# showlab/VideoSwap

Measured on NVIDIA H100. Metric: denoise-steps/sec, 16f 512^2 SD1.5 UNet3D (CFG UNet fwd + CFG combine + DDIM step), higher is better.
Workload: dtype f16

## Files before the change

### videoswap_b200/csrc/attention_tc.cu

```cuda
#include "common.cuh"
#include "kernels.h"

namespace vs {
namespace {

constexpr int TQ = 64;
constexpr int ATT_THREADS = 384;
constexpr int PRODUCER_REGS = 24, CONSUMER_REGS = 240;

template <int D>
struct TCfg {
  static constexpr int BKV = 128;
  static constexpr int STAGES = D > 64 ? 3 : 4;
  static constexpr int NCB = (D + 63) / 64;
  static constexpr int DPK = (D + 15) / 16 * 16;
  static constexpr int Q_BLOCK = TQ * 128;
  static constexpr int KV_BLOCK = BKV * 128;
  static constexpr int Q_BYTES = NCB * Q_BLOCK;
  static constexpr int KV_STAGE_BYTES = 2 * NCB * KV_BLOCK;
  static constexpr int OREG = (D > 64) ? 32 + 8 : 32;
  static constexpr int SMEM = 2 * Q_BYTES + STAGES * KV_STAGE_BYTES + 1024 + 8 * (1 + 2 * STAGES);
  static_assert(D == 40 || D == 80, "head dims of the tensor-core path");
  static_assert(SMEM <= 227 * 1024, "shared memory");
};

struct TAttnArgs {
  CUtensorMap tmQ, tmK, tmV;
  __half* o;
  int ldo;
  long long o_bs;
  int nq, nk, kv_div;
  float scale_log2;
};

__device__ __forceinline__ float fast_exp2(float x) {
  float y;
  asm("ex2.approx.ftz.f32 %0, %1;" : "=f"(y) : "f"(x));
  return y;
}
__device__ __forceinline__ uint32_t pack_h2(float a, float b) {
  const __half2 h = __floats2half2_rn(a, b);
  return *reinterpret_cast<const uint32_t*>(&h);
}

template <int D>
__global__ void __launch_bounds__(ATT_THREADS, 1) attn_tc_kernel(const __grid_constant__ TAttnArgs p) {
  using C = TCfg<D>;
  constexpr int BKV = C::BKV, STAGES = C::STAGES;
  extern __shared__ uint8_t smem_raw[];
  const uint32_t base = (smem_u32(smem_raw) + 1023u) & ~1023u;
  const uint32_t q_s = base;
  const uint32_t kv_s = q_s + 2 * C::Q_BYTES;
  const uint32_t bars = kv_s + STAGES * C::KV_STAGE_BYTES;
  const uint32_t q_full = bars;
  auto kv_full = [&](int s) { return bars + 8u * (1 + s); };
  auto kv_empty = [&](int s) { return bars + 8u * (1 + STAGES + s); };

  const int warp = threadIdx.x >> 5, lane = threadIdx.x & 31, wg = threadIdx.x >> 7;
  const int q0 = blockIdx.x * 2 * TQ, head = blockIdx.y, b = blockIdx.z;
  const int nkt = (p.nk + BKV - 1) / BKV;

  if (threadIdx.x == 0) {
    prefetch_tmap(&p.tmQ); prefetch_tmap(&p.tmK); prefetch_tmap(&p.tmV);
    mbar_init(q_full, 1);
    for (int s = 0; s < STAGES; ++s) {
      mbar_init(kv_full(s), 1);
      mbar_init(kv_empty(s), 8);
    }
    fence_barrier_init();
  }
  __syncthreads();
  pdl_trigger();
  pdl_wait();

  if (wg == 0) {
    setmaxnreg_dec<PRODUCER_REGS>();
    if (warp != 0) return;
    const int bk = b / p.kv_div;
    if (elect_one()) {
      mbar_expect_tx(q_full, 2 * C::Q_BYTES);
#pragma unroll
      for (int g = 0; g < 2; ++g)
#pragma unroll
        for (int cb = 0; cb < C::NCB; ++cb)
          tma_load_4d(q_s + g * C::Q_BYTES + cb * C::Q_BLOCK, &p.tmQ, q_full, cb * 64, head, q0 + g * TQ, b);
    }
    __syncwarp();
    for (int j = 0, s = 0, ph = 0; j < nkt; ++j) {
      mbar_wait(kv_empty(s), ph ^ 1);
      if (elect_one()) {
        const uint32_t k_dst = kv_s + s * C::KV_STAGE_BYTES, v_dst = k_dst + C::NCB * C::KV_BLOCK;
        mbar_expect_tx(kv_full(s), C::KV_STAGE_BYTES);
#pragma unroll
        for (int cb = 0; cb < C::NCB; ++cb) {
          tma_load_4d(k_dst + cb * C::KV_BLOCK, &p.tmK, kv_full(s), cb * 64, head, j * BKV, bk);
          tma_load_4d(v_dst + cb * C::KV_BLOCK, &p.tmV, kv_full(s), cb * 64, head, j * BKV, bk);
        }
      }
      __syncwarp();
      if (++s == STAGES) { s = 0; ph ^= 1; }
    }
    return;
  }

  setmaxnreg_inc<CONSUMER_REGS>();
  const int g = wg - 1, wq = warp & 3, q4 = lane & 3;
  const uint32_t qg = q_s + g * C::Q_BYTES;
  const int bar_mine = 1 + g, bar_other = 2 - g;
  if (g == 1) named_bar_arrive(bar_other, 256);

  const float sc = p.scale_log2;
  float o[C::OREG];
#pragma unroll
  for (int i = 0; i < C::OREG; ++i) o[i] = 0.f;
  float m[2] = {-INFINITY, -INFINITY}, l[2] = {0.f, 0.f};
  float s[BKV / 2];
  uint32_t pf[BKV / 16][4];

  auto stage_addr = [&](int j) { return kv_s + (uint32_t)(j % STAGES) * C::KV_STAGE_BYTES; };
  auto issue_qk = [&](int j) {
    const uint32_t k_a = stage_addr(j);
#pragma unroll
    for (int k = 0; k < C::DPK / 16; ++k) {
      const uint32_t qoff = (uint32_t)((k * 16) / 64) * C::Q_BLOCK + (uint32_t)((k * 16) % 64) * 2;
      const uint32_t koff = (uint32_t)((k * 16) / 64) * C::KV_BLOCK + (uint32_t)((k * 16) % 64) * 2;
      wgmma_ss<BKV>(s, gmma_desc_sw128(qg + qoff), gmma_desc_sw128(k_a + koff), k != 0 ? 1u : 0u);
    }
  };
  auto issue_pv = [&](int j) {
    const uint32_t v_a = stage_addr(j) + C::NCB * C::KV_BLOCK;
#pragma unroll
    for (int kk = 0; kk < BKV / 16; ++kk) {
      const uint32_t v_rows = v_a + kk * 16 * 128;
      wgmma_m64n64_rs<1>(o, pf[kk], gmma_desc_sw128_mn(v_rows, C::KV_BLOCK), 1u);
      if (D > 64) wgmma_m64n16_rs<1>(o + 32, pf[kk], gmma_desc_sw128_mn(v_rows + C::KV_BLOCK, C::KV_BLOCK), 1u);
    }
  };
  auto softmax = [&](int j, float* alpha) {
    const int kbase = j * BKV;
    if (kbase + BKV > p.nk) {
#pragma unroll
      for (int i = 0; i < BKV / 2; ++i)
        if (kbase + 8 * (i >> 2) + 2 * q4 + (i & 1) >= p.nk) s[i] = -INFINITY;
    }
#pragma unroll
    for (int h = 0; h < 2; ++h) {
      float mx = m[h];
#pragma unroll
      for (int i = 2 * h; i < BKV / 2; i += 4) mx = fmaxf(mx, fmaxf(s[i], s[i + 1]));
      mx = fmaxf(mx, __shfl_xor_sync(0xffffffffu, mx, 1));
      mx = fmaxf(mx, __shfl_xor_sync(0xffffffffu, mx, 2));
      alpha[h] = fast_exp2((m[h] - mx) * sc);
      m[h] = mx;
      const float ms = mx * sc;
      float rs = 0.f;
#pragma unroll
      for (int i = 2 * h; i < BKV / 2; i += 4) {
        s[i] = fast_exp2(fmaf(s[i], sc, -ms));
        s[i + 1] = fast_exp2(fmaf(s[i + 1], sc, -ms));
        rs += s[i] + s[i + 1];
      }
      l[h] = fmaf(l[h], alpha[h], rs);
    }
  };
  auto pack_p = [&]() {
#pragma unroll
    for (int kk = 0; kk < BKV / 16; ++kk)
#pragma unroll
      for (int r = 0; r < 4; ++r) pf[kk][r] = pack_h2(s[8 * kk + 2 * r], s[8 * kk + 2 * r + 1]);
  };
  auto release = [&](int j) {
    if (lane == 0) mbar_arrive(kv_empty(j % STAGES));
  };

  mbar_wait(q_full, 0);
  mbar_wait(kv_full(0), 0);
  named_bar_sync(bar_mine, 256);
  wgmma_fence();
  issue_qk(0);
  wgmma_commit();
  named_bar_arrive(bar_other, 256);
  wgmma_wait<0>();
  {
    float alpha[2];
    softmax(0, alpha);
    pack_p();
  }
  for (int j = 1; j < nkt; ++j) {
    mbar_wait(kv_full(j % STAGES), (j / STAGES) & 1);
    named_bar_sync(bar_mine, 256);
    wgmma_fence();
    issue_qk(j);
    wgmma_commit();
    issue_pv(j - 1);
    wgmma_commit();
    named_bar_arrive(bar_other, 256);
    wgmma_wait<1>();
    float alpha[2];
    softmax(j, alpha);
    if (p.kv_div > 0) wgmma_wait<0>();
    release(j - 1);
#pragma unroll
    for (int i = 0; i < C::OREG; ++i) o[i] *= alpha[(i >> 1) & 1];
    pack_p();
  }
  named_bar_sync(bar_mine, 256);
  wgmma_fence();
  issue_pv(nkt - 1);
  wgmma_commit();
  if (g == 0) named_bar_arrive(bar_other, 256);
  wgmma_wait<0>();
  release(nkt - 1);

#pragma unroll
  for (int h = 0; h < 2; ++h) {
    l[h] += __shfl_xor_sync(0xffffffffu, l[h], 1);
    l[h] += __shfl_xor_sync(0xffffffffu, l[h], 2);
  }
  const float inv[2] = {1.f / l[0], 1.f / l[1]};
  const int r0 = q0 + g * TQ + 16 * wq + (lane >> 2);
  __half* ob = p.o + b * p.o_bs + head * D;
#pragma unroll
  for (int i = 0; i < C::OREG; i += 2) {
    const int h = (i >> 1) & 1, c = 8 * (i >> 2) + 2 * q4, r = r0 + 8 * h;
    if (c < D && r < p.nq)
      *reinterpret_cast<__half2*>(ob + (long long)r * p.ldo + c) = __floats2half2_rn(o[i] * inv[h], o[i + 1] * inv[h]);
  }
}

template <int D>
int launch(cudaStream_t st, const __half* q, int ldq, const __half* k, int ldk, const __half* v, int ldv, __half* o, int ldo,
           int batch, int nq, int nk, int heads, long long q_bs, long long kv_bs, long long o_bs, int kv_div) {
  using C = TCfg<D>;
  static bool configured = false;
  if (!configured) {
    VS_CHECK_CUDA(cudaFuncSetAttribute(attn_tc_kernel<D>, cudaFuncAttributeMaxDynamicSharedMemorySize, C::SMEM));
    configured = true;
  }
  TAttnArgs a;
  memset(&a, 0, sizeof(a));
  const int bkv = (batch + kv_div - 1) / kv_div;
  {
    const uint64_t dims[4] = {(uint64_t)D, (uint64_t)heads, (uint64_t)nq, (uint64_t)batch};
    const uint64_t str[3] = {(uint64_t)D * 2, (uint64_t)ldq * 2, (uint64_t)(q_bs > 0 ? q_bs : (long long)nq * ldq) * 2};
    const uint32_t box[4] = {64, 1, TQ, 1};
    if (make_tmap_f16(&a.tmQ, q, 4, dims, str, box, 1)) return 3;
  }
  {
    const uint64_t dims[4] = {(uint64_t)D, (uint64_t)heads, (uint64_t)nk, (uint64_t)bkv};
    const uint64_t strk[3] = {(uint64_t)D * 2, (uint64_t)ldk * 2, (uint64_t)(kv_bs > 0 ? kv_bs : (long long)nk * ldk) * 2};
    const uint64_t strv[3] = {(uint64_t)D * 2, (uint64_t)ldv * 2, (uint64_t)(kv_bs > 0 ? kv_bs : (long long)nk * ldv) * 2};
    const uint32_t box[4] = {64, 1, (uint32_t)C::BKV, 1};
    if (make_tmap_f16(&a.tmK, k, 4, dims, strk, box, 1)) return 3;
    if (make_tmap_f16(&a.tmV, v, 4, dims, strv, box, 1)) return 3;
  }
  a.o = o; a.ldo = ldo; a.o_bs = o_bs; a.nq = nq; a.nk = nk; a.kv_div = kv_div;
  a.scale_log2 = 1.4426950408889634f / sqrtf((float)D);
  ProfScope prof(st, PC_ATTN, 4.0 * batch * heads * (double)nq * nk * D, 1, nq, nk, D);
  dim3 grid((nq + 2 * TQ - 1) / (2 * TQ), heads, batch);
  return launch_pdl(attn_tc_kernel<D>, grid, dim3(ATT_THREADS), C::SMEM, st, 1, a);
}

}

int attention_tc(cudaStream_t st, const __half* q, int ldq, const __half* k, int ldk, const __half* v, int ldv, __half* o,
                 int ldo, int batch, int nq, int nk, int heads, int d, long long q_bs, long long kv_bs, long long o_bs,
                 int kv_div) {
  if ((ldq % 8) || (ldk % 8) || (ldv % 8) || (ldo % 2)) return -1;
  if ((q_bs % 8) || (kv_bs % 8)) return -1;
  VS_REQUIRE(kv_div >= 1, "attention_tc: kv_div must be >= 1 (got %d)", kv_div);
  if (d == 40) return launch<40>(st, q, ldq, k, ldk, v, ldv, o, ldo, batch, nq, nk, heads, q_bs, kv_bs, o_bs, kv_div);
  if (d == 80) return launch<80>(st, q, ldq, k, ldk, v, ldv, o, ldo, batch, nq, nk, heads, q_bs, kv_bs, o_bs, kv_div);
  return -1;
}

}
```

### videoswap_b200/csrc/common.cuh

```cuda
#pragma once
#include <cuda.h>
#include <cuda_fp16.h>
#include <cuda_runtime.h>
#include <stdint.h>
#include <stdio.h>

namespace vs {

void set_error(const char* fmt, ...);
const char* last_error();

#define VS_CHECK_CUDA(expr)                                                                         \
  do {                                                                                              \
    cudaError_t _e = (expr);                                                                        \
    if (_e != cudaSuccess) {                                                                        \
      vs::set_error("%s:%d CUDA error %s: %s", __FILE__, __LINE__, #expr, cudaGetErrorString(_e)); \
      return 1;                                                                                     \
    }                                                                                               \
  } while (0)

#define VS_REQUIRE(cond, ...)                \
  do {                                       \
    if (!(cond)) {                           \
      vs::set_error(__VA_ARGS__);            \
      return 2;                              \
    }                                        \
  } while (0)

int make_tmap_f16(CUtensorMap* out, const void* base, int rank, const uint64_t* dims, const uint64_t* strides_bytes,
                  const uint32_t* box, int swizzle );

int num_sms();
int get_option(const char* name);

#ifdef __CUDACC__
template <typename... KArgs, typename... Args>
int launch_pdl(void (*kernel)(KArgs...), dim3 grid, dim3 block, size_t smem, cudaStream_t st, int cluster_x, Args&&... args) {
  cudaLaunchConfig_t cfg = {};
  cfg.gridDim = grid;
  cfg.blockDim = block;
  cfg.dynamicSmemBytes = smem;
  cfg.stream = st;
  cudaLaunchAttribute attr[2];
  int n = 0;
  if (get_option("pdl") != 0) {
    attr[n].id = cudaLaunchAttributeProgrammaticStreamSerialization;
    attr[n].val.programmaticStreamSerializationAllowed = 1;
    ++n;
  }
  if (cluster_x > 1) {
    attr[n].id = cudaLaunchAttributeClusterDimension;
    attr[n].val.clusterDim.x = cluster_x;
    attr[n].val.clusterDim.y = 1;
    attr[n].val.clusterDim.z = 1;
    ++n;
  }
  cfg.attrs = attr;
  cfg.numAttrs = n;
  VS_CHECK_CUDA(cudaLaunchKernelEx(&cfg, kernel, static_cast<KArgs>(args)...));
  return 0;
}
#endif

enum ProfCat { PC_GEMM = 0, PC_CONV = 1, PC_ATTN = 2, PC_TATTN = 3, PC_GROUPNORM = 4, PC_LAYERNORM = 5, PC_OTHER = 6, PC_COUNT = 7 };
struct ProfScope {
  ProfScope(cudaStream_t st, int cat, double work, int nlaunch = 1, long long m = 0, int n = 0, int k = 0);
  ~ProfScope();
  cudaStream_t st_; int idx_;
};
void prof_enable(bool on);
void prof_reset();
int prof_collect(int cat, double* ms, double* work, long long* count);
int prof_dump(const char* path);
long long launch_count();
void count_launch(int n);

#ifdef __CUDACC__
__device__ __forceinline__ uint32_t smem_u32(const void* p) { return (uint32_t)__cvta_generic_to_shared(p); }

__device__ __forceinline__ void mbar_init(uint32_t bar, uint32_t count) {
  asm volatile("mbarrier.init.shared::cta.b64 [%0], %1;" ::"r"(bar), "r"(count) : "memory");
}
__device__ __forceinline__ void fence_barrier_init() {
  asm volatile("fence.mbarrier_init.release.cluster;" ::: "memory");
}
__device__ __forceinline__ void fence_proxy_async() { asm volatile("fence.proxy.async.shared::cta;" ::: "memory"); }
__device__ __forceinline__ void mbar_expect_tx(uint32_t bar, uint32_t bytes) {
  asm volatile("mbarrier.arrive.expect_tx.shared::cta.b64 _, [%0], %1;" ::"r"(bar), "r"(bytes) : "memory");
}
__device__ __forceinline__ void mbar_arrive(uint32_t bar) {
  asm volatile("mbarrier.arrive.shared::cta.b64 _, [%0];" ::"r"(bar) : "memory");
}
__device__ __forceinline__ bool mbar_try_wait(uint32_t bar, uint32_t parity) {
  uint32_t ok;
  asm volatile(
      "{\n\t.reg .pred p;\n\t"
      "mbarrier.try_wait.parity.shared::cta.b64 p, [%1], %2;\n\t"
      "selp.u32 %0, 1, 0, p;\n\t}"
      : "=r"(ok)
      : "r"(bar), "r"(parity)
      : "memory");
  return ok != 0;
}
__device__ __forceinline__ void mbar_wait(uint32_t bar, uint32_t parity) {
  if (mbar_try_wait(bar, parity)) return;
  uint32_t spins = 0;
  while (!mbar_try_wait(bar, parity)) {
    if (++spins > (1u << 25)) __trap();
  }
}

__device__ __forceinline__ void prefetch_tmap(const CUtensorMap* m) {
  asm volatile("prefetch.tensormap [%0];" ::"l"(reinterpret_cast<uint64_t>(m)) : "memory");
}
__device__ __forceinline__ void tma_load_2d(uint32_t dst, const CUtensorMap* m, uint32_t bar, int c0, int c1) {
  asm volatile(
      "cp.async.bulk.tensor.2d.shared::cluster.global.mbarrier::complete_tx::bytes [%0], [%1, {%3, %4}], [%2];"
      ::"r"(dst), "l"(reinterpret_cast<uint64_t>(m)), "r"(bar), "r"(c0), "r"(c1)
      : "memory");
}
__device__ __forceinline__ void bulk_load(uint32_t dst, const void* src, uint32_t bytes, uint32_t bar) {
  asm volatile(
      "cp.async.bulk.shared::cluster.global.mbarrier::complete_tx::bytes [%0], [%1], %2, [%3];"
      ::"r"(dst), "l"(reinterpret_cast<uint64_t>(src)), "r"(bytes), "r"(bar)
      : "memory");
}
__device__ __forceinline__ void tma_load_4d(uint32_t dst, const CUtensorMap* m, uint32_t bar, int c0, int c1, int c2,
                                            int c3) {
  asm volatile(
      "cp.async.bulk.tensor.4d.shared::cluster.global.mbarrier::complete_tx::bytes [%0], [%1, {%3, %4, %5, %6}], [%2];"
      ::"r"(dst), "l"(reinterpret_cast<uint64_t>(m)), "r"(bar), "r"(c0), "r"(c1), "r"(c2), "r"(c3)
      : "memory");
}

__device__ __forceinline__ bool elect_one() {
  uint32_t pred;
  asm volatile(
      "{\n\t.reg .pred P;\n\t"
      "elect.sync _|P, 0xffffffff;\n\t"
      "selp.u32 %0, 1, 0, P;\n\t}"
      : "=r"(pred));
  return pred != 0;
}

__device__ __forceinline__ uint32_t cluster_ctarank() {
  uint32_t r;
  asm volatile("mov.u32 %0, %%cluster_ctarank;" : "=r"(r));
  return r;
}
__device__ __forceinline__ void cluster_sync_all() {
  asm volatile("barrier.cluster.arrive.release.aligned;" ::: "memory");
  asm volatile("barrier.cluster.wait.acquire.aligned;" ::: "memory");
}
__device__ __forceinline__ uint32_t mapa_shared(uint32_t addr, uint32_t rank) {
  uint32_t r;
  asm volatile("mapa.shared::cluster.u32 %0, %1, %2;" : "=r"(r) : "r"(addr), "r"(rank));
  return r;
}
__device__ __forceinline__ void named_bar_sync(int id, int nthreads) {
  asm volatile("bar.sync %0, %1;" ::"r"(id), "r"(nthreads) : "memory");
}
__device__ __forceinline__ void named_bar_arrive(int id, int nthreads) {
  asm volatile("bar.arrive %0, %1;" ::"r"(id), "r"(nthreads) : "memory");
}

__device__ __forceinline__ void pdl_trigger() { asm volatile("griddepcontrol.launch_dependents;" ::: "memory"); }
__device__ __forceinline__ void pdl_wait() { asm volatile("griddepcontrol.wait;" ::: "memory"); }

template <int N>
__device__ __forceinline__ void setmaxnreg_dec() { asm volatile("setmaxnreg.dec.sync.aligned.u32 %0;" ::"n"(N)); }
template <int N>
__device__ __forceinline__ void setmaxnreg_inc() { asm volatile("setmaxnreg.inc.sync.aligned.u32 %0;" ::"n"(N)); }

__device__ __forceinline__ void wgmma_fence() { asm volatile("wgmma.fence.sync.aligned;" ::: "memory"); }
__device__ __forceinline__ void wgmma_commit() { asm volatile("wgmma.commit_group.sync.aligned;" ::: "memory"); }
template <int N>
__device__ __forceinline__ void wgmma_wait() { asm volatile("wgmma.wait_group.sync.aligned %0;" ::"n"(N) : "memory"); }

__device__ __forceinline__ uint64_t gmma_desc_sw128(uint32_t smem_addr) {
  uint64_t d = 0;
  d |= (uint64_t)((smem_addr & 0x3FFFF) >> 4);
  d |= (uint64_t)1 << 16;
  d |= (uint64_t)(1024 >> 4) << 32;
  d |= (uint64_t)1 << 62;
  return d;
}
__device__ __forceinline__ uint64_t gmma_desc_sw128_mn(uint32_t smem_addr, uint32_t lbo_bytes) {
  uint64_t d = 0;
  d |= (uint64_t)((smem_addr & 0x3FFFF) >> 4);
  d |= (uint64_t)((lbo_bytes >> 4) & 0x3FFF) << 16;
  d |= (uint64_t)(1024 >> 4) << 32;
  d |= (uint64_t)1 << 62;
  return d;
}

#define VS_R8(i) "+f"(d[i]), "+f"(d[i + 1]), "+f"(d[i + 2]), "+f"(d[i + 3]), "+f"(d[i + 4]), "+f"(d[i + 5]), "+f"(d[i + 6]), "+f"(d[i + 7])
template <int N>
__device__ __forceinline__ void wgmma_ss(float* d, uint64_t da, uint64_t db, uint32_t scale_d);
#define VS_REGS_0_31 "%0,%1,%2,%3,%4,%5,%6,%7,%8,%9,%10,%11,%12,%13,%14,%15,%16,%17,%18,%19,%20,%21,%22,%23,%24,%25,%26,%27,%28,%29,%30,%31"
#define VS_REGS_32_63 "%32,%33,%34,%35,%36,%37,%38,%39,%40,%41,%42,%43,%44,%45,%46,%47,%48,%49,%50,%51,%52,%53,%54,%55,%56,%57,%58,%59,%60,%61,%62,%63"
#define VS_REGS_64_79 "%64,%65,%66,%67,%68,%69,%70,%71,%72,%73,%74,%75,%76,%77,%78,%79"
#define VS_REGS_80_127 "%80,%81,%82,%83,%84,%85,%86,%87,%88,%89,%90,%91,%92,%93,%94,%95,%96,%97,%98,%99,%100,%101,%102,%103,%104,%105,%106,%107,%108,%109,%110,%111,%112,%113,%114,%115,%116,%117,%118,%119,%120,%121,%122,%123,%124,%125,%126,%127"
#define VS_WGMMA_SS(N, REGS, IA, IB, IS, ...)                                                                     \
  template <>                                                                                                     \
  __device__ __forceinline__ void wgmma_ss<N>(float* d, uint64_t da, uint64_t db, uint32_t scale_d) {           \
    asm volatile("{\n\t.reg .pred p;\n\tsetp.ne.b32 p, %" #IS ", 0;\n\t"                                         \
                 "wgmma.mma_async.sync.aligned.m64n" #N "k16.f32.f16.f16 {" REGS "}, %" #IA ", %" #IB ", p, 1, 1, 0, 0;\n\t}" \
                 : __VA_ARGS__                                                                                    \
                 : "l"(da), "l"(db), "r"(scale_d));                                                               \
  }
VS_WGMMA_SS(64, VS_REGS_0_31, 32, 33, 34, VS_R8(0), VS_R8(8), VS_R8(16), VS_R8(24))
VS_WGMMA_SS(128, VS_REGS_0_31 "," VS_REGS_32_63, 64, 65, 66, VS_R8(0), VS_R8(8), VS_R8(16), VS_R8(24), VS_R8(32), VS_R8(40),
            VS_R8(48), VS_R8(56))
VS_WGMMA_SS(160, VS_REGS_0_31 "," VS_REGS_32_63 "," VS_REGS_64_79, 80, 81, 82, VS_R8(0), VS_R8(8), VS_R8(16), VS_R8(24),
            VS_R8(32), VS_R8(40), VS_R8(48), VS_R8(56), VS_R8(64), VS_R8(72))
VS_WGMMA_SS(256, VS_REGS_0_31 "," VS_REGS_32_63 "," VS_REGS_64_79 "," VS_REGS_80_127, 128, 129, 130, VS_R8(0), VS_R8(8),
            VS_R8(16), VS_R8(24), VS_R8(32), VS_R8(40), VS_R8(48), VS_R8(56), VS_R8(64), VS_R8(72), VS_R8(80), VS_R8(88),
            VS_R8(96), VS_R8(104), VS_R8(112), VS_R8(120))
#undef VS_WGMMA_SS
#undef VS_REGS_0_31
#undef VS_REGS_32_63
#undef VS_REGS_64_79
#undef VS_REGS_80_127
template <int TB = 0>
__device__ __forceinline__ void wgmma_m64n16(float* d, uint64_t da, uint64_t db, uint32_t scale_d) {
  asm volatile(
      "{\n\t.reg .pred p;\n\tsetp.ne.b32 p, %10, 0;\n\t"
      "wgmma.mma_async.sync.aligned.m64n16k16.f32.f16.f16 {%0,%1,%2,%3,%4,%5,%6,%7}, %8, %9, p, 1, 1, 0, %11;\n\t}"
      : VS_R8(0)
      : "l"(da), "l"(db), "r"(scale_d), "n"(TB));
}
template <int TB = 0>
__device__ __forceinline__ void wgmma_m64n64_rs(float* d, const uint32_t* a, uint64_t db, uint32_t scale_d) {
  asm volatile(
      "{\n\t.reg .pred p;\n\tsetp.ne.b32 p, %37, 0;\n\t"
      "wgmma.mma_async.sync.aligned.m64n64k16.f32.f16.f16 "
      "{%0,%1,%2,%3,%4,%5,%6,%7,%8,%9,%10,%11,%12,%13,%14,%15,%16,%17,%18,%19,%20,%21,%22,%23,%24,%25,%26,%27,%28,%29,%30,%31}, "
      "{%32,%33,%34,%35}, %36, p, 1, 1, %38;\n\t}"
      : VS_R8(0), VS_R8(8), VS_R8(16), VS_R8(24)
      : "r"(a[0]), "r"(a[1]), "r"(a[2]), "r"(a[3]), "l"(db), "r"(scale_d), "n"(TB));
}
template <int TB = 0>
__device__ __forceinline__ void wgmma_m64n16_rs(float* d, const uint32_t* a, uint64_t db, uint32_t scale_d) {
  asm volatile(
      "{\n\t.reg .pred p;\n\tsetp.ne.b32 p, %13, 0;\n\t"
      "wgmma.mma_async.sync.aligned.m64n16k16.f32.f16.f16 {%0,%1,%2,%3,%4,%5,%6,%7}, {%8,%9,%10,%11}, %12, p, 1, 1, %14;\n\t}"
      : VS_R8(0)
      : "r"(a[0]), "r"(a[1]), "r"(a[2]), "r"(a[3]), "l"(db), "r"(scale_d), "n"(TB));
}
#undef VS_R8

__device__ __forceinline__ float silu_f(float x) { return __fdividef(x, 1.f + __expf(-x)); }
__device__ __forceinline__ float gelu_erf_f(float x) { return 0.5f * x * (1.f + erff(x * 0.70710678118654752f)); }
__device__ __forceinline__ float gelu_erf_fast(float x) {
  const float z = fabsf(x) * 0.70710678118654752f;
  float t;
  asm("rcp.approx.ftz.f32 %0, %1;" : "=f"(t) : "f"(fmaf(0.3275911f, z, 1.f)));
  float poly = fmaf(1.061405429f, t, -1.453152027f);
  poly = fmaf(poly, t, 1.421413741f);
  poly = fmaf(poly, t, -0.284496736f);
  poly = fmaf(poly, t, 0.254829592f);
  poly *= t;
  float e;
  asm("ex2.approx.ftz.f32 %0, %1;" : "=f"(e) : "f"(-1.4426950408889634f * z * z));
  const float erf_abs = fmaf(-poly, e, 1.f);
  const float erf_s = copysignf(erf_abs, x);
  return 0.5f * x * (1.f + erf_s);
}
__device__ __forceinline__ float gelu_sig(float x) {
  const float xn = fmaxf(x, -5.f);
  const float xc = fminf(xn, 5.f);
  const float u = xc * xc;
  float q = fmaf(u, 2.47135360e-05f, 7.37690930e-04f);
  q = fmaf(q, u, -1.05988323e-01f);
  q = fmaf(q, u, -2.30164247e+00f);
  float e;
  asm("ex2.approx.ftz.f32 %0, %1;" : "=f"(e) : "f"(xc * q));
  return __fdividef(xn, 1.f + e);
}
__device__ __forceinline__ float quick_gelu_f(float v) {
  const float t = fminf(-2.4554669595930157f * v, 64.f);
  float e;
  asm("ex2.approx.ftz.f32 %0, %1;" : "=f"(e) : "f"(t));
  return __fdividef(v, 1.f + e);
}
#endif

}
```

Before: 11.28.

## Add persistent short-key attention kernel with resident KV and TMA output stores

Adds a dedicated attention kernel for key lengths up to 128, such as the 16-frame temporal attention and the 77-token cross-attention. Each persistent CTA loads the whole K/V tile once and keeps it in shared memory while streaming many Q tiles through a 6-stage pipeline. It does a single-pass softmax with no online rescaling and writes outputs via shared memory and TMA bulk stores. For D=40 it also uses an n40 wgmma for PV instead of n64, cutting wasted MMA columns and accumulator registers. This removes the multi-tile KV pipeline overhead and under-filled launches for short sequences, at the cost of more templated kernel instances and extra barrier complexity.

Result: no change. 11.36, median of 6 (+0.8%).

```diff
diff --git a/videoswap_b200/csrc/attention_tc.cu b/videoswap_b200/csrc/attention_tc.cu
--- a/videoswap_b200/csrc/attention_tc.cu
+++ b/videoswap_b200/csrc/attention_tc.cu
@@ -18,7 +18,7 @@
   static constexpr int KV_BLOCK = BKV * 128;
   static constexpr int Q_BYTES = NCB * Q_BLOCK;
   static constexpr int KV_STAGE_BYTES = 2 * NCB * KV_BLOCK;
-  static constexpr int OREG = (D > 64) ? 32 + 8 : 32;
+  static constexpr int OREG = (D > 64) ? 32 + 8 : 20;
   static constexpr int SMEM = 2 * Q_BYTES + STAGES * KV_STAGE_BYTES + 1024 + 8 * (1 + 2 * STAGES);
   static_assert(D == 40 || D == 80, "head dims of the tensor-core path");
   static_assert(SMEM <= 227 * 1024, "shared memory");
@@ -41,6 +41,15 @@
 __device__ __forceinline__ uint32_t pack_h2(float a, float b) {
   const __half2 h = __floats2half2_rn(a, b);
   return *reinterpret_cast<const uint32_t*>(&h);
+}
+template <int D>
+__device__ __forceinline__ void pv_k16(float* o, const uint32_t* a, uint32_t v_rows, uint32_t kv_block) {
+  if (D == 40) {
+    wgmma_m64n40_rs<1>(o, a, gmma_desc_sw128_mn(v_rows, kv_block), 1u);
+  } else {
+    wgmma_m64n64_rs<1>(o, a, gmma_desc_sw128_mn(v_rows, kv_block), 1u);
+    wgmma_m64n16_rs<1>(o + 32, a, gmma_desc_sw128_mn(v_rows + kv_block, kv_block), 1u);
+  }
 }
 
 template <int D>
@@ -132,8 +141,7 @@
 #pragma unroll
     for (int kk = 0; kk < BKV / 16; ++kk) {
       const uint32_t v_rows = v_a + kk * 16 * 128;
-      wgmma_m64n64_rs<1>(o, pf[kk], gmma_desc_sw128_mn(v_rows, C::KV_BLOCK), 1u);
-      if (D > 64) wgmma_m64n16_rs<1>(o + 32, pf[kk], gmma_desc_sw128_mn(v_rows + C::KV_BLOCK, C::KV_BLOCK), 1u);
+      pv_k16<D>(o, pf[kk], v_rows, C::KV_BLOCK);
     }
   };
   auto softmax = [&](int j, float* alpha) {
@@ -228,8 +236,259 @@
   }
 }
 
+constexpr int SHORT_THREADS = 288;
+constexpr int SHORT_PRODUCER_WARP = 8;
+
+template <int D, int KT>
+struct SCfg {
+  static constexpr int NCB = TCfg<D>::NCB, DPK = TCfg<D>::DPK, OREG = TCfg<D>::OREG;
+  static constexpr int QST = 6;
+  static constexpr int MIN_CTAS = (D > 64 || KT > 112) ? 1 : 2;
+  static constexpr int Q_BLOCK = TQ * 128;
+  static constexpr int Q_STAGE = NCB * Q_BLOCK;
+  static constexpr int KV_BLOCK = KT * 128;
+  static constexpr int KV_BYTES = 2 * NCB * KV_BLOCK;
+  static constexpr int O_BYTES = TQ * D * 2;
+  static constexpr int SMEM = KV_BYTES + QST * Q_STAGE + 2 * O_BYTES + 1024 + 8 * (2 + 2 * QST);
+  static_assert(KT % 16 == 0 && KT <= TCfg<D>::BKV, "key tile");
+  static_assert(SMEM <= 227 * 1024, "shared memory");
+};
+
+struct SAttnArgs {
+  CUtensorMap tmQ, tmK, tmV, tmO;
+  int nqb, batch, nbk, kv_div, nk, items;
+  float scale_log2;
+};
+
+template <int D, int KT>
+__global__ void __launch_bounds__(SHORT_THREADS, SCfg<D, KT>::MIN_CTAS) attn_short_kernel(const __grid_constant__ SAttnArgs p) {
+  using C = SCfg<D, KT>;
+  constexpr int QST = C::QST;
+  extern __shared__ uint8_t smem_raw[];
+  const uint32_t base = (smem_u32(smem_raw) + 1023u) & ~1023u;
+  const uint32_t k_s = base, v_s = base + C::NCB * C::KV_BLOCK;
+  const uint32_t q_s = base + C::KV_BYTES;
+  const uint32_t o_s = q_s + QST * C::Q_STAGE;
+  const uint32_t bars = o_s + 2 * C::O_BYTES;
+  const uint32_t kv_full = bars, kv_empty = bars + 8;
+  auto q_full = [&](int s) { return bars + 8u * (2 + s); };
+  auto q_empty = [&](int s) { return bars + 8u * (2 + QST + s); };
+
+  const int warp = threadIdx.x >> 5, lane = threadIdx.x & 31;
+  const int t0 = (int)((long long)blockIdx.x * p.items / gridDim.x);
+  const int n = (int)((long long)(blockIdx.x + 1) * p.items / gridDim.x) - t0;
+
+  if (threadIdx.x == 0) {
+    prefetch_tmap(&p.tmQ); prefetch_tmap(&p.tmK); prefetch_tmap(&p.tmV); prefetch_tmap(&p.tmO);
+    mbar_init(kv_full, 1);
+    mbar_init(kv_empty, 8);
+    for (int s = 0; s < QST; ++s) {
+      mbar_init(q_full(s), 1);
+      mbar_init(q_empty(s), 4);
+    }
+    fence_barrier_init();
+  }
+  __syncthreads();
+  pdl_trigger();
+  pdl_wait();
+
+  auto decode = [&](int t, int& head, int& b, int& q0) {
+    const int r = t / p.nqb;
+    q0 = (t - r * p.nqb) * TQ;
+    head = r / p.batch;
+    b = r - head * p.batch;
+  };
+
+  if (warp == SHORT_PRODUCER_WARP) {
+    int gen = -1, key = -1;
+    for (int i = 0; i < n; ++i) {
+      int head, b, q0;
+      decode(t0 + i, head, b, q0);
+      const int bk = b / p.kv_div;
+      if (head * p.nbk + bk != key) {
+        key = head * p.nbk + bk;
+        ++gen;
+        mbar_wait(kv_empty, (gen & 1) ^ 1);
+        if (elect_one()) {
+          mbar_expect_tx(kv_full, C::KV_BYTES);
+#pragma unroll
+          for (int cb = 0; cb < C::NCB; ++cb) {
+            tma_load_4d(k_s + cb * C::KV_BLOCK, &p.tmK, kv_full, cb * 64, head, 0, bk);
+            tma_load_4d(v_s + cb * C::KV_BLOCK, &p.tmV, kv_full, cb * 64, head, 0, bk);
+          }
+        }
+        __syncwarp();
+      }
+      const int s = i % QST;
+      mbar_wait(q_empty(s), ((i / QST) & 1) ^ 1);
+      if (elect_one()) {
+        mbar_expect_tx(q_full(s), C::Q_STAGE);
+#pragma unroll
+        for (int cb = 0; cb < C::NCB; ++cb)
+          tma_load_4d(q_s + s * C::Q_STAGE + cb * C::Q_BLOCK, &p.tmQ, q_full(s), cb * 64, head, q0, b);
+      }
+      __syncwarp();
+    }
+    return;
+  }
+
+  const int g = warp >> 2, wq = warp & 3, q4 = lane & 3, tid = threadIdx.x & 127;
+  const uint32_t og = o_s + g * C::O_BYTES;
+  const float sc = p.scale_log2;
+  int gen = -1, key = -1;
+  for (int i = 0; i < n; ++i) {
+    int head, b, q0;
+    decode(t0 + i, head, b, q0);
+    const int bk = b / p.kv_div;
+    if (head * p.nbk + bk != key) {
+      if (gen >= 0 && lane == 0) mbar_arrive(kv_empty);
+      key = head * p.nbk + bk;
+      ++gen;
+      mbar_wait(kv_full, gen & 1);
+    }
+    if ((i & 1) != g) continue;
+    const int st = i % QST;
+    const uint32_t qa = q_s + st * C::Q_STAGE;
+    mbar_wait(q_full(st), (i / QST) & 1);
+
+    float s[KT / 2];
+    wgmma_fence();
+#pragma unroll
+    for (int k = 0; k < C::DPK / 16; ++k) {
+      const uint32_t off_q = (uint32_t)((k * 16) / 64) * C::Q_BLOCK + (uint32_t)((k * 16) % 64) * 2;
+      const uint32_t off_k = (uint32_t)((k * 16) / 64) * C::KV_BLOCK + (uint32_t)((k * 16) % 64) * 2;
+      wgmma_ss<KT>(s, gmma_desc_sw128(qa + off_q), gmma_desc_sw128(k_s + off_k), k != 0 ? 1u : 0u);
+    }
+    wgmma_commit();
+    wgmma_wait<0>();
+    if (lane == 0) mbar_arrive(q_empty(st));
+
+    if (KT > p.nk) {
+#pragma unroll
+      for (int j = 0; j < KT / 2; ++j)
+        if (8 * (j >> 2) + 2 * q4 + (j & 1) >= p.nk) s[j] = -INFINITY;
+    }
+    float l[2];
+#pragma unroll
+    for (int h = 0; h < 2; ++h) {
+      float mx = -INFINITY;
+#pragma unroll
+      for (int j = 2 * h; j < KT / 2; j += 4) mx = fmaxf(mx, fmaxf(s[j], s[j + 1]));
+      mx = fmaxf(mx, __shfl_xor_sync(0xffffffffu, mx, 1));
+      mx = fmaxf(mx, __shfl_xor_sync(0xffffffffu, mx, 2));
+      const float ms = mx * sc;
+      float rs = 0.f;
+#pragma unroll
+      for (int j = 2 * h; j < KT / 2; j += 4) {
+        s[j] = fast_exp2(fmaf(s[j], sc, -ms));
+        s[j + 1] = fast_exp2(fmaf(s[j + 1], sc, -ms));
+        rs += s[j] + s[j + 1];
+      }
+      l[h] = rs;
+    }
+    uint32_t pf[KT / 16][4];
+#pragma unroll
+    for (int kk = 0; kk < KT / 16; ++kk)
+#pragma unroll
+      for (int r = 0; r < 4; ++r) pf[kk][r] = pack_h2(s[8 * kk + 2 * r], s[8 * kk + 2 * r + 1]);
+
+    float o[C::OREG];
+#pragma unroll
+    for (int j = 0; j < C::OREG; ++j) o[j] = 0.f;
+    wgmma_fence();
+#pragma unroll
+    for (int kk = 0; kk < KT / 16; ++kk) {
+      const uint32_t v_rows = v_s + kk * 16 * 128;
+      pv_k16<D>(o, pf[kk], v_rows, C::KV_BLOCK);
+    }
+    wgmma_commit();
+    wgmma_wait<0>();
+
+#pragma unroll
+    for (int h = 0; h < 2; ++h) {
+      l[h] += __shfl_xor_sync(0xffffffffu, l[h], 1);
+      l[h] += __shfl_xor_sync(0xffffffffu, l[h], 2);
+    }
+    const float inv[2] = {1.f / l[0], 1.f / l[1]};
+    if (tid == 0) bulk_wait_read<0>();
+    named_bar_sync(1 + g, 128);
+    const int r0 = 16 * wq + (lane >> 2);
+#pragma unroll
+    for (int j = 0; j < C::OREG; j += 2) {
+      const int h = (j >> 1) & 1, c = 8 * (j >> 2) + 2 * q4;
+      if (c < D) {
+        const __half2 v2 = __floats2half2_rn(o[j] * inv[h], o[j + 1] * inv[h]);
+        asm volatile("st.shared.b32 [%0], %1;" ::"r"(og + (uint32_t)(((r0 + 8 * h) * D + c) * 2)),
+                     "r"(*reinterpret_cast<const uint32_t*>(&v2)) : "memory");
+      }
+    }
+    fence_proxy_async();
+    named_bar_sync(1 + g, 128);
+    if (tid == 0) {
+      tma_store_4d(&p.tmO, og, 0, head, q0, b);
+      bulk_commit();
+    }
+  }
+  if (gen >= 0 && lane == 0) mbar_arrive(kv_empty);
+  if (tid == 0) bulk_wait<0>();
+}
+
+template <int D, int KT>
+int launch_short(cudaStream_t st, const CUtensorMap& tmQ, const __half* k, int ldk, const __half* v, int ldv, __half* o,
+                 int ldo, int batch, int nq, int nk, int heads, long long kv_bs, long long o_bs, int kv_div) {
+  using C = SCfg<D, KT>;
+  static int ctas_per_sm = 0;
+  if (ctas_per_sm == 0) {
+    VS_CHECK_CUDA(cudaFuncSetAttribute(attn_short_kernel<D, KT>, cudaFuncAttributeMaxDynamicSharedMemorySize, C::SMEM));
+    VS_CHECK_CUDA(cudaOccupancyMaxActiveBlocksPerMultiprocessor(&ctas_per_sm, attn_short_kernel<D, KT>, SHORT_THREADS,
+                                                                C::SMEM));
+    VS_REQUIRE(ctas_per_sm > 0, "attention_tc: short-key kernel does not fit on an SM");
+  }
+  SAttnArgs a;
+  memset(&a, 0, sizeof(a));
+  a.tmQ = tmQ;
+  const int bkv = (batch + kv_div - 1) / kv_div;
+  {
+    const uint64_t dims[4] = {(uint64_t)D, (uint64_t)heads, (uint64_t)nk, (uint64_t)bkv};
+    const uint64_t strk[3] = {(uint64_t)D * 2, (uint64_t)ldk * 2, (uint64_t)(kv_bs > 0 ? kv_bs : (long long)nk * ldk) * 2};
+    const uint64_t strv[3] = {(uint64_t)D * 2, (uint64_t)ldv * 2, (uint64_t)(kv_bs > 0 ? kv_bs : (long long)nk * ldv) * 2};
+    const uint32_t box[4] = {64, 1, (uint32_t)KT, 1};
+    if (make_tmap_f16(&a.tmK, k, 4, dims, strk, box, 1)) return 3;
+    if (make_tmap_f16(&a.tmV, v, 4, dims, strv, box, 1)) return 3;
+  }
+  {
+    const uint64_t dims[4] = {(uint64_t)D, (uint64_t)heads, (uint64_t)nq, (uint64_t)batch};
+    const uint64_t str[3] = {(uint64_t)D * 2, (uint64_t)ldo * 2, (uint64_t)o_bs * 2};
+    const uint32_t box[4] = {(uint32_t)D, 1, TQ, 1};
+    if (make_tmap_f16(&a.tmO, o, 4, dims, str, box, 0)) return 3;
+  }
+  a.nqb = (nq + TQ - 1) / TQ;
+  a.batch = batch; a.nbk = bkv; a.kv_div = kv_div; a.nk = nk;
+  const long long items = (long long)heads * batch * a.nqb;
+  VS_REQUIRE(items < (1LL << 31), "attention_tc: too many work items (%lld)", items);
+  a.items = (int)items;
+  a.scale_log2 = 1.4426950408889634f / sqrtf((float)D);
+  ProfScope prof(st, PC_ATTN, 4.0 * batch * heads * (double)nq * nk * D, 1, nq, nk, D);
+  const long long cap = (long long)num_sms() * ctas_per_sm;
+  const int grid = (int)(items < cap ? items : cap);
+  return launch_pdl(attn_short_kernel<D, KT>, dim3(grid), dim3(SHORT_THREADS), C::SMEM, st, 1, a);
+}
+
 template <int D>
-int launch(cudaStream_t st, const __half* q, int ldq, const __half* k, int ldk, const __half* v, int ldv, __half* o, int ldo,
+int launch_short_nk(cudaStream_t st, const CUtensorMap& tmQ, const __half* k, int ldk, const __half* v, int ldv, __half* o,
+                    int ldo, int batch, int nq, int nk, int heads, long long kv_bs, long long o_bs, int kv_div) {
+  switch ((nk + 15) / 16) {
+#define VS_SHORT(T)                                                                                                   \
+  case T:                                                                                                             \
+    return launch_short<D, 16 * T>(st, tmQ, k, ldk, v, ldv, o, ldo, batch, nq, nk, heads, kv_bs, o_bs, kv_div);
+    VS_SHORT(1) VS_SHORT(2) VS_SHORT(3) VS_SHORT(4) VS_SHORT(5) VS_SHORT(6) VS_SHORT(7) VS_SHORT(8)
+#undef VS_SHORT
+  }
+  VS_REQUIRE(false, "attention_tc: short-key path got nk = %d", nk);
+}
+
+template <int D>
+int launch(cudaStream_t st,const __half* q, int ldq, const __half* k, int ldk, const __half* v, int ldv, __half* o, int ldo,
            int batch, int nq, int nk, int heads, long long q_bs, long long kv_bs, long long o_bs, int kv_div) {
   using C = TCfg<D>;
   static bool configured = false;
@@ -246,6 +505,8 @@
     const uint32_t box[4] = {64, 1, TQ, 1};
     if (make_tmap_f16(&a.tmQ, q, 4, dims, str, box, 1)) return 3;
   }
+  if (nk <= C::BKV && ldo % 8 == 0 && o_bs % 8 == 0 && (reinterpret_cast<uintptr_t>(o) & 15) == 0)
+    return launch_short_nk<D>(st, a.tmQ, k, ldk, v, ldv, o, ldo, batch, nq, nk, heads, kv_bs, o_bs, kv_div);
   {
     const uint64_t dims[4] = {(uint64_t)D, (uint64_t)heads, (uint64_t)nk, (uint64_t)bkv};
     const uint64_t strk[3] = {(uint64_t)D * 2, (uint64_t)ldk * 2, (uint64_t)(kv_bs > 0 ? kv_bs : (long long)nk * ldk) * 2};
diff --git a/videoswap_b200/csrc/common.cuh b/videoswap_b200/csrc/common.cuh
--- a/videoswap_b200/csrc/common.cuh
+++ b/videoswap_b200/csrc/common.cuh
@@ -132,6 +132,16 @@
       ::"r"(dst), "l"(reinterpret_cast<uint64_t>(m)), "r"(bar), "r"(c0), "r"(c1), "r"(c2), "r"(c3)
       : "memory");
 }
+__device__ __forceinline__ void tma_store_4d(const CUtensorMap* m, uint32_t src, int c0, int c1, int c2, int c3) {
+  asm volatile("cp.async.bulk.tensor.4d.global.shared::cta.bulk_group [%0, {%2, %3, %4, %5}], [%1];"
+               ::"l"(reinterpret_cast<uint64_t>(m)), "r"(src), "r"(c0), "r"(c1), "r"(c2), "r"(c3)
+               : "memory");
+}
+__device__ __forceinline__ void bulk_commit() { asm volatile("cp.async.bulk.commit_group;" ::: "memory"); }
+template <int N>
+__device__ __forceinline__ void bulk_wait_read() { asm volatile("cp.async.bulk.wait_group.read %0;" ::"n"(N) : "memory"); }
+template <int N>
+__device__ __forceinline__ void bulk_wait() { asm volatile("cp.async.bulk.wait_group %0;" ::"n"(N) : "memory"); }
 
 __device__ __forceinline__ bool elect_one() {
   uint32_t pred;
@@ -209,7 +219,27 @@
                  : __VA_ARGS__                                                                                    \
                  : "l"(da), "l"(db), "r"(scale_d));                                                               \
   }
+#define VS_REGS_0_7 "%0,%1,%2,%3,%4,%5,%6,%7"
+#define VS_REGS_8_15 "%8,%9,%10,%11,%12,%13,%14,%15"
+#define VS_REGS_16_23 "%16,%17,%18,%19,%20,%21,%22,%23"
+#define VS_REGS_32_39 "%32,%33,%34,%35,%36,%37,%38,%39"
+#define VS_REGS_40_47 "%40,%41,%42,%43,%44,%45,%46,%47"
+#define VS_REGS_48_55 "%48,%49,%50,%51,%52,%53,%54,%55"
+VS_WGMMA_SS(16, VS_REGS_0_7, 8, 9, 10, VS_R8(0))
+VS_WGMMA_SS(32, VS_REGS_0_7 "," VS_REGS_8_15, 16, 17, 18, VS_R8(0), VS_R8(8))
+VS_WGMMA_SS(48, VS_REGS_0_7 "," VS_REGS_8_15 "," VS_REGS_16_23, 24, 25, 26, VS_R8(0), VS_R8(8), VS_R8(16))
 VS_WGMMA_SS(64, VS_REGS_0_31, 32, 33, 34, VS_R8(0), VS_R8(8), VS_R8(16), VS_R8(24))
+VS_WGMMA_SS(80, VS_REGS_0_31 "," VS_REGS_32_39, 40, 41, 42, VS_R8(0), VS_R8(8), VS_R8(16), VS_R8(24), VS_R8(32))
+VS_WGMMA_SS(96, VS_REGS_0_31 "," VS_REGS_32_39 "," VS_REGS_40_47, 48, 49, 50, VS_R8(0), VS_R8(8), VS_R8(16), VS_R8(24),
+            VS_R8(32), VS_R8(40))
+VS_WGMMA_SS(112, VS_REGS_0_31 "," VS_REGS_32_39 "," VS_REGS_40_47 "," VS_REGS_48_55, 56, 57, 58, VS_R8(0), VS_R8(8),
+            VS_R8(16), VS_R8(24), VS_R8(32), VS_R8(40), VS_R8(48))
+#undef VS_REGS_0_7
+#undef VS_REGS_8_15
+#undef VS_REGS_16_23
+#undef VS_REGS_32_39
+#undef VS_REGS_40_47
+#undef VS_REGS_48_55
 VS_WGMMA_SS(128, VS_REGS_0_31 "," VS_REGS_32_63, 64, 65, 66, VS_R8(0), VS_R8(8), VS_R8(16), VS_R8(24), VS_R8(32), VS_R8(40),
             VS_R8(48), VS_R8(56))
 VS_WGMMA_SS(160, VS_REGS_0_31 "," VS_REGS_32_63 "," VS_REGS_64_79, 80, 81, 82, VS_R8(0), VS_R8(8), VS_R8(16), VS_R8(24),
@@ -238,6 +268,16 @@
       "{%0,%1,%2,%3,%4,%5,%6,%7,%8,%9,%10,%11,%12,%13,%14,%15,%16,%17,%18,%19,%20,%21,%22,%23,%24,%25,%26,%27,%28,%29,%30,%31}, "
       "{%32,%33,%34,%35}, %36, p, 1, 1, %38;\n\t}"
       : VS_R8(0), VS_R8(8), VS_R8(16), VS_R8(24)
+      : "r"(a[0]), "r"(a[1]), "r"(a[2]), "r"(a[3]), "l"(db), "r"(scale_d), "n"(TB));
+}
+template <int TB = 0>
+__device__ __forceinline__ void wgmma_m64n40_rs(float* d, const uint32_t* a, uint64_t db, uint32_t scale_d) {
+  asm volatile(
+      "{\n\t.reg .pred p;\n\tsetp.ne.b32 p, %25, 0;\n\t"
+      "wgmma.mma_async.sync.aligned.m64n40k16.f32.f16.f16 "
+      "{%0,%1,%2,%3,%4,%5,%6,%7,%8,%9,%10,%11,%12,%13,%14,%15,%16,%17,%18,%19}, "
+      "{%20,%21,%22,%23}, %24, p, 1, 1, %26;\n\t}"
+      : VS_R8(0), VS_R8(8), "+f"(d[16]), "+f"(d[17]), "+f"(d[18]), "+f"(d[19])
       : "r"(a[0]), "r"(a[1]), "r"(a[2]), "r"(a[3]), "l"(db), "r"(scale_d), "n"(TB));
 }
 template <int TB = 0>
```
